# lilijiangg/AutoDiffusion

Measured on AMD Instinct MI355X. Metric: images/sec (node), ADM-G ImageNet-64 4-step DDIM, higher is better.
Workload: dtype bf16

## Files before the change

### autodiffusion_amd/csrc/adm_conv.hip

```cpp
#include <stdlib.h>

#include <type_traits>

#include "adm_common.h"
#include "adm_conv_internal.h"

namespace {

typedef __attribute__((ext_vector_type(4))) unsigned int u32x4;

constexpr int KC = 32;
constexpr int ROWB = 64 + 32;
constexpr int TI_MAX = 4;
constexpr unsigned OOB = 0x80000000u;

struct ConvK {
  const uint16_t* in0; const uint16_t* in1; const uint16_t* w; const uint16_t* res;
  const float* bias; const float* aa; const float* ab; void* out;
  float* stats;
  int stat_slabs;
  int N, H, W, C0, C1, Cout;
  int TH, TW, TI, tiles_x, tiles_y;
  int tw_shift, thw_shift;
  unsigned rcp_hpi, rcp_hw2;
  int out_mode;
  int in_up, res_up;
  int ntiles16, nblocks_n;
  int total_tiles;
  unsigned wbytes;
  int ksplit, cps;
  float* ws;
  int tap_mask, ooy, oox, slab_off;
  int nph, nbp;
  unsigned phase_bytes;
  const uint16_t* f0; const uint16_t* f1;
  int FC0, FC1;
  float out_scale;
};

template <int BM>
constexpr int stat_groups() { return BM == 128 ? 2 : 1; }

template <int NT, int HALO>
constexpr int halo_slots() { return ((HALO * 4 + NT - 1) / NT) * NT / 4; }
template <int NT, int HALO>
constexpr int conv_smem_bytes_k() { return 2 * halo_slots<NT, HALO>() * ROWB + 2 * TI_MAX * 64 * 4; }
template <int NT, int BN, int HALO, int BM>
constexpr int conv_smem_bytes() {
  constexpr int k = conv_smem_bytes_k<NT, HALO>();
  constexpr int e = BM * (BN * 2 + 16);
  constexpr int r = NT * 64;
  return (k > e ? k : e) > r ? (k > e ? k : e) : r;
}
// ... 63 lines not shown
  const int wave = __builtin_amdgcn_readfirstlane(tid >> 6);
  const int wm = wave / WN, wn = wave % WN;
  const int lc = lane & 15, lq = lane >> 4;

  const int xcd = blockIdx.x & 7;
  const int gx = (int)(gridDim.x >> 3) + (xcd < (int)(gridDim.x & 7));
  const int tcount = (p.total_tiles >> 3) + (xcd < (p.total_tiles & 7));
  const int tstart = xcd * (p.total_tiles >> 3) + min(xcd, p.total_tiles & 7);
  int tl = blockIdx.x >> 3;
  if (tl >= tcount) return;

  const int HW2 = p.TW + 2 * PAD;
  const int HPI = (p.TH + 2 * PAD) * HW2;
  const int HP = p.TI * HPI;
  const int Cin = p.C0 + p.C1;
  const int HWimg = p.H * p.W;
  const int chunks = Cin / KC;
  const int c0chunks = p.C0 / KC;
  const __amdgpu_buffer_rsrc_t rsw = __builtin_amdgcn_make_buffer_rsrc((void*)p.w, 0, p.wbytes, 0x00020000);
  const __amdgpu_buffer_rsrc_t rsb = __builtin_amdgcn_make_buffer_rsrc((void*)p.bias, 0, p.Cout * 4, 0x00020000);

  unsigned ti_pack = 0;
#pragma unroll
  for (int ps = 0; ps < PASSES; ++ps) {
    const int hp = (tid + ps * NT) >> SEGSH;
    if (hp < HP) ti_pack |= (unsigned)(hp / HPI) << (4 * ps);
  }
  const int seg = tid & (SEGP - 1);
  const int hslot = (tid >> SEGSH) * ROWB + seg * 16;

  const int alane = ((lc / p.TW) * HW2 + lc % p.TW) * ROWB + lq * 16;
  int aoff[TM];
#pragma unroll
  for (int i = 0; i < TM; ++i) {
    const int m0 = (wm * TM + i) * 16;
    const int ti = m0 / (p.TH * p.TW), rem = m0 % (p.TH * p.TW);
    aoff[i] = (ti * HPI + (rem / p.TW) * HW2) * ROWB;
  }
  const unsigned wstep = (unsigned)p.ntiles16 * 1024u;

  int nb = 0, mt = 0, img0 = 0, y0 = 0, x0 = 0;
  [[maybe_unused]] int ph = p.slab_off;
  int sp = 0, cb = 0, ce = chunks;
  __amdgpu_buffer_rsrc_t rs0 = rsw, rs1 = rsw;
  [[maybe_unused]] __amdgpu_buffer_rsrc_t rs2 = rsw, rs3 = rsw;
  int pixrel[PASSES];
  unsigned wofs[TN];
  typedef __attribute__((address_space(3))) void* lds_ptr_t;
  auto tile_origin = [&](int lt, int& nb_, int& mt_, int& img0_, int& y0_, int& x0_) {
    if (p.ksplit > 1) {
      sp = lt % p.ksplit;
      lt /= p.ksplit;
      cb = sp * p.cps;
      ce = cb + p.cps;
    }
    nb_ = lt % p.nblocks_n;
    mt_ = lt / p.nblocks_n;
    if constexpr (UPPH) {
      if (p.nph > 1) { ph = nb_ / p.nbp; nb_ -= ph * p.nbp; }
    }
    if (p.TI == 1) {
      const int per_img = p.tiles_x * p.tiles_y;
      img0_ = mt_ / per_img;
      const int r = mt_ % per_img;
      y0_ = (r / p.tiles_x) * p.TH;
      x0_ = (r % p.tiles_x) * p.TW;
    } else {
      img0_ = mt_ * p.TI;
      y0_ = 0;
      x0_ = 0;
    }
  };
  auto tile_setup = [&]() {
    const int nimg = min(p.TI, p.N - img0);
    const int Hs = p.H >> p.in_up, Ws = p.W >> p.in_up;
    rs0 = __builtin_amdgcn_make_buffer_rsrc((void*)(p.in0 + (long long)img0 * Hs * Ws * p.C0), 0, nimg * Hs * Ws * p.C0 * 2, 0x00020000);
    rs1 = __builtin_amdgcn_make_buffer_rsrc((void*)(p.C1 ? p.in1 + (long long)img0 * HWimg * p.C1 : p.in0), 0,
                                            p.C1 ? nimg * HWimg * p.C1 * 2 : 0, 0x00020000);
    if constexpr (FOLD) {
      rs2 = __builtin_amdgcn_make_buffer_rsrc((void*)(p.f0 + (long long)img0 * HWimg * p.FC0), 0, nimg * HWimg * p.FC0 * 2, 0x00020000);
      rs3 = __builtin_amdgcn_make_buffer_rsrc((void*)(p.FC1 ? p.f1 + (long long)img0 * HWimg * p.FC1 : p.f0), 0,
                                              p.FC1 ? nimg * HWimg * p.FC1 * 2 : 0, 0x00020000);
    }
    int tid_s = tid;
    asm volatile("" : "+v"(tid_s));
#pragma unroll
    for (int ps = 0; ps < PASSES; ++ps) {
      const int hp = (tid_s + ps * NT) >> SEGSH;
      const int ti = (int)(((unsigned)hp * p.rcp_hpi) >> 20), rem = hp - ti * HPI;
      const int ry = (int)(((unsigned)rem * p.rcp_hw2) >> 20), rx = rem - ry * HW2;
      const int y = y0 + ry - PAD, x = x0 + rx - PAD;
      const int ok = (int)(hp < HP) & (int)(ti < nimg) & (int)(y >= 0) & (int)(y < p.H) & (int)(x >= 0) & (int)(x < p.W);
      pixrel[ps] = ok ? (ti * Hs + (y >> p.in_up)) * Ws + (x >> p.in_up) : -1;
    }
    const int seg_s = tid_s & (SEGP - 1), lane_s = tid_s & 63;
    {
      const bool first = cb < c0chunks;
      const int cs = first ? p.C0 : p.C1, co = (first ? cb : cb - c0chunks) * KC;
      const __amdgpu_buffer_rsrc_t rsf = first ? rs0 : rs1;
#pragma unroll
      for (int ps = 0; ps < PASSES; ++ps) {
        const unsigned voff = pixrel[ps] >= 0 ? (unsigned)(pixrel[ps] * cs + co + seg_s * 8) * 2u : OOB;
        __builtin_amdgcn_raw_ptr_buffer_load_lds(rsf, (lds_ptr_t)(halo + (ps * NT + wave * 64) * 16), 16, (int)voff, 0, 0, 0);
      }
    }
    if constexpr (PRO != 0 && !ONEW) {
      if (wave < 2) {
        const int half = wave, idx = lane_s;
        const __amdgpu_buffer_rsrc_t rsa = __builtin_amdgcn_make_buffer_rsrc((void*)(half == 0 ? p.aa : p.ab), 0, p.N * Cin * 4, 0x00020000);
        const int buf = idx / (TI_MAX * (KC / 4)), ti = (idx / (KC / 4)) % TI_MAX, part = idx % (KC / 4);
        const int n = min(img0 + ti, p.N - 1);
        const unsigned voff = ti < p.TI ? (unsigned)(n * Cin + min(cb + buf, ce - 1) * KC + part * 4) * 4u : OOB;
        __builtin_amdgcn_raw_ptr_buffer_load_lds(rsa, (lds_ptr_t)(abuf + half * (2 * TI_MAX * KC)), 16, (int)voff, 0, 0, 0);
      }
    }
#pragma unroll
    for (int j = 0; j < TN; ++j) {
      const int tile = nb * (BN / 16) + wn * TN + j;
      wofs[j] = tile < p.ntiles16 ? (unsigned)((tile * 64 + lane) * 16) + (UPPH ? (unsigned)ph * p.phase_bytes : 0u) : OOB;
    }
  };

  f32x4 acc[TM][TN];

  auto halo_load = [&](int c, int ps) -> uint4 {
    const bool first = c < c0chunks;
    const int cs = first ? p.C0 : p.C1, co = (first ? c : c - c0chunks) * KC;
    const __amdgpu_buffer_rsrc_t rs = first ? rs0 : rs1;
    const unsigned voff = pixrel[ps] >= 0 ? (unsigned)(pixrel[ps] * cs + co + seg * 8) * 2u : OOB;
    return bufload16(rs, voff, 0);
  };
  [[maybe_unused]] auto halo_load_pad = [&](int c, int lastc, int ps) -> uint4 {
    const int cc = min(c, lastc);
    const bool first = cc < c0chunks;
// ... 104 lines not shown
#pragma unroll
    for (int i = 0; i < AFD; ++i) __builtin_amdgcn_sched_group_barrier(0x100, 1, 0);
#pragma unroll
    for (int i = 0; i < TM; ++i) {
      if (i + AFD < TM) __builtin_amdgcn_sched_group_barrier(0x100, 1, 0);
      __builtin_amdgcn_sched_group_barrier(0x008, TN, 0);
    }
  };

  constexpr bool NOEXIT = TM == 4 && !COLD;
  constexpr int WRING = T3 ? 3 : 4;
  uint4 wr[WRING][TN];
  constexpr int RINGN = (TAPS == 1 && NOEXIT) ? 4 : 2;
  uint4 ring[RINGN][PASSES];
  float4 bs[TN];
  auto first_loads = [&](int lq_) {
    const int last = ce - 1;
    if constexpr (T3) {
      load_w(cb * 9, wr[0]);
      load_w(cb * 9 + 1, wr[1]);
    } else {
      load_w(cb, wr[0]);
      load_w(NOEXIT ? cb + 1 : min(cb + 1, last), wr[1]);
      load_w(NOEXIT ? cb + 2 : min(cb + 2, last), wr[2]);
#pragma unroll
      for (int ps = 0; ps < PASSES; ++ps) ring[1][ps] = NOEXIT ? halo_load_pad(cb + 1, last, ps) : halo_load(min(cb + 1, last), ps);
      if constexpr (RINGN > 2) {
#pragma unroll
        for (int q = 2; q < RINGN; ++q) {
#pragma unroll
          for (int ps = 0; ps < PASSES; ++ps) ring[q][ps] = NOEXIT ? halo_load_pad(cb + q, last, ps) : halo_load(min(cb + q, last), ps);
        }
      }
    }
    if constexpr (ONEW) affine_regs(cb, img0);
#pragma unroll
    for (int j = 0; j < TN; ++j) {
      const int bch = nb * BN + (wn * TN + j) * 16 + lq_ * 4;
      const uint4 b = bufload16(rsb, (bch + 3 < p.Cout && p.ksplit <= 1) ? (unsigned)bch * 4u : OOB, 0);
      bs[j] = make_float4(__uint_as_float(b.x), __uint_as_float(b.y), __uint_as_float(b.z), __uint_as_float(b.w));
    }
  };
  auto first_park = [&]() {
    uint4 raw[PASSES];
#pragma unroll
    for (int ps = 0; ps < PASSES; ++ps) raw[ps] = *reinterpret_cast<const uint4*>(halo + (ps * NT + tid) * 16);
    __syncthreads();
#pragma unroll
    for (int ps = 0; ps < PASSES; ++ps) halo_write(raw[ps], ps, 0);
  };

  int ltile = tstart + tl;
  tile_origin(ltile, nb, mt, img0, y0, x0);
  tile_setup();
  first_loads(lq);
  __syncthreads();
  first_park();

  for (;;) {
    ADM_TSTAMP(ltile, 0);
#pragma unroll
    for (int i = 0; i < TM; ++i)
#pragma unroll
      for (int j = 0; j < TN; ++j) acc[i][j] = f32x4{bs[j].x, bs[j].y, bs[j].z, bs[j].w};
    __syncthreads();
    ADM_TSTAMP(ltile, 1);

    const int tnext = tl + gx;
    const bool more = tnext < tcount;
    if constexpr (T3 && ONEW) {
// ... 108 lines not shown
              if constexpr (RAWNEXT) raw_write(hprev, t - 1, hb ^ 1);
              else halo_write(hprev, t - 1, hb ^ 1);
            }
          }
          hprev = hcur;
          if (!UPPH || (((0x1b << ((ph >> 1) * 3 + (ph & 1))) >> t) & 1))
            mfma_tap(halo + hb * Lds::HB + ((t / 3) * HW2 + (t % 3)) * ROWB, wr[t % 3]);
        }
        __syncthreads();
      };
      for (int c = cb; c + 1 < ce; ++c) chunk(c, std::true_type{}, std::false_type{});
      if constexpr (!FOLD) {
        chunk(ce - 1, std::false_type{}, std::false_type{});
      } else {
        chunk(ce - 1, std::true_type{}, std::true_type{});
        const int fch = (p.FC0 + p.FC1) / KC, flast = fch - 1;
        const int fstep0 = chunks * 9;
        const unsigned char* const hc = halo + (HW2 + 1) * ROWB;
        constexpr int CPASS = BM * SEGP / NT;
        static_assert(CPASS * NT == BM * SEGP && CPASS <= PASSES, "centre staging: whole passes");
        int cpix[CPASS], cslot[CPASS];
        {
          int tid_c = tid;
          asm volatile("" : "+v"(tid_c));
          const int nimg_c = min(p.TI, p.N - img0);
#pragma unroll
          for (int ps = 0; ps < CPASS; ++ps) {
            const int pp = (tid_c + ps * NT) >> SEGSH;
            const int ti = pp >> p.thw_shift, rem = pp & ((1 << p.thw_shift) - 1);
            const int py = rem >> p.tw_shift, px = rem & (p.TW - 1);
            cpix[ps] = ti < nimg_c ? (ti * p.H + y0 + py) * p.W + x0 + px : -1;
            cslot[ps] = (ti * HPI + (py + 1) * HW2 + px + 1) * ROWB + (tid_c & (SEGP - 1)) * 16;
          }
        }
        auto cload = [&](int k, int ps) -> uint4 {
          const int f0chunks = p.FC0 / KC;
          const bool first = k < f0chunks;
          const int cs = first ? p.FC0 : p.FC1, co = (first ? k : k - f0chunks) * KC;
          const __amdgpu_buffer_rsrc_t rs = first ? rs2 : rs3;
          const unsigned voff = cpix[ps] >= 0 ? (unsigned)(cpix[ps] * cs + co + seg * 8) * 2u : OOB;
          return bufload16(rs, voff, 0);
        };
#pragma unroll
        for (int q = 1; q <= RINGN; ++q) {
#pragma unroll
          for (int ps = 0; ps < CPASS; ++ps) ring[q % RINGN][ps] = cload(min(q, flast), ps);
        }
        auto fbody = [&](int j, auto s_) {
          constexpr int S = decltype(s_)::value;
          if (j > flast) return;
          const int buf = (ce + j) & 1;
          load_w(fstep0 + min(j + 2, flast), wr[(S + 2) % 3]);
          mfma_tap(hc + buf * Lds::HB, wr[S % 3]);
#pragma unroll
          for (int ps = 0; ps < CPASS; ++ps) *reinterpret_cast<uint4*>(halo + (buf ^ 1) * Lds::HB + cslot[ps]) = ring[(S + 1) % RINGN][ps];
// ... 36 lines not shown
        body(c0 + 3, I1{}, I3{});
      }
    }
    ADM_TSTAMP(ltile, 2);

    const int ltile_done = ltile;
    (void)ltile_done;
    if (!COLD || (p.out_mode == 0 && p.ksplit <= 1)) {
      constexpr int EROW = BN * 2 + 16;
      constexpr int SEGS = BN / 8;
      constexpr int PR = NT / SEGS;
      constexpr int RG = BM / SGROUPS;
      constexpr int NIT = (RG + PR - 1) / PR;
      int tid_e = tid;
      asm volatile("" : "+v"(tid_e));
      const int sg = tid_e % SEGS, prow = tid_e / SEGS;
      const int gch = nb * BN + sg * 8;
      const bool act = prow < PR && gch < p.Cout;
      const int thw_mask = (1 << p.thw_shift) - 1, tw_mask = (1 << p.tw_shift) - 1;
      const long long ebase = UPPH ? (((long long)img0 * (2 * p.H) + 2 * y0 + (ph >> 1)) * (2 * p.W) + 2 * x0 + (ph & 1)) * p.Cout + gch
                                   : (((long long)img0 * p.H + y0) * p.W + x0) * p.Cout + gch;
      uint16_t* const obase = reinterpret_cast<uint16_t*>(p.out) + ebase;
      const int Hr = p.H >> p.res_up, Wr = p.W >> p.res_up;
      const uint16_t* const rbase = p.res ? p.res + (((long long)img0 * Hr + (y0 >> p.res_up)) * Wr + (x0 >> p.res_up)) * p.Cout + gch : nullptr;
      const int img0_d = img0;
      float* sdst[SGROUPS];
#pragma unroll
      for (int g = 0; g < SGROUPS; ++g) {
        const int n = img0 + ((g * RG) >> p.thw_shift);
        const int slab = p.TI == 1 ? (UPPH ? (mt % (p.tiles_x * p.tiles_y)) * 4 + ph : (mt % (p.tiles_x * p.tiles_y)) * SGROUPS + g) : 0;
        sdst[g] = (p.stats && tid_e < BN && nb * BN + tid_e < p.Cout && n < p.N)
                      ? p.stats + (((long long)n * p.stat_slabs + slab) * p.Cout + nb * BN + tid_e) * 2 : nullptr;
      }
      ADM_TSTAMP(ltile_done, 10);
#pragma unroll
      for (int j = 0; j < TN; ++j) {
        const int ch0 = (wn * TN + j) * 16 + lq * 4;
#pragma unroll
        for (int i = 0; i < TM; ++i) {
          uint2 o;
          o.x = adm_pack2(acc[i][j][0], acc[i][j][1]);
          o.y = adm_pack2(acc[i][j][2], acc[i][j][3]);
          *reinterpret_cast<uint2*>(stg + ((wm * TM + i) * 16 + lc) * EROW + ch0 * 2) = o;
        }
      }
      ADM_TSTAMP(ltile_done, 11);
      if (more) {
        tl = tnext;
        ltile = tstart + tl;
        tile_origin(ltile, nb, mt, img0, y0, x0);
        tile_setup();
      }
      int eoff[SGROUPS][NIT];
#pragma unroll
      for (int g = 0; g < SGROUPS; ++g)
#pragma unroll
        for (int k = 0; k < NIT; ++k) {
          const int ml = prow + k * PR, m = g * RG + ml;
          const int ti = m >> p.thw_shift, rem = m & thw_mask;
          eoff[g][k] = (act && ml < RG && img0_d + ti < p.N)
                           ? (UPPH ? ((rem >> p.tw_shift) * (4 * p.W) + 2 * (rem & tw_mask)) * p.Cout
                                   : ((ti * p.H + (rem >> p.tw_shift)) * p.W + (rem & tw_mask)) * p.Cout)
                           : -1;
        }
      ADM_TSTAMP(ltile_done, 12);
      uint4 rr[SGROUPS][NIT];
#pragma unroll
      for (int g = 0; g < SGROUPS; ++g)
#pragma unroll
        for (int k = 0; k < NIT; ++k) {
          rr[g][k] = make_uint4(0, 0, 0, 0);
          if (rbase && eoff[g][k] >= 0) {
            const int m = g * RG + prow + k * PR;
            const int ti = m >> p.thw_shift, rem = m & thw_mask;
            const int roff = ((ti * Hr + ((rem >> p.tw_shift) >> p.res_up)) * Wr + ((rem & tw_mask) >> p.res_up)) * p.Cout;
            rr[g][k] = *reinterpret_cast<const uint4*>(rbase + roff);
          }
        }
      [[maybe_unused]] float ga[8], gb[8];
      if constexpr (GNB) {
        const long long ao = (long long)img0_d * p.Cout + gch;
        if (act) {
          *reinterpret_cast<float4*>(ga) = *reinterpret_cast<const float4*>(p.aa + ao);
          *reinterpret_cast<float4*>(ga + 4) = *reinterpret_cast<const float4*>(p.aa + ao + 4);
          *reinterpret_cast<float4*>(gb) = *reinterpret_cast<const float4*>(p.ab + ao);
          *reinterpret_cast<float4*>(gb + 4) = *reinterpret_cast<const float4*>(p.ab + ao + 4);
        } else {
#pragma unroll
          for (int e = 0; e < 8; ++e) { ga[e] = 0.f; gb[e] = 0.f; }
        }
      }
      if (more) first_loads((tid_e & 63) >> 4);
      ADM_TSTAMP(ltile_done, 13);
      __syncthreads();
      ADM_TSTAMP(ltile_done, 3);
      if (more) first_park();
      ADM_TSTAMP(ltile_done, 4);
      typedef float f32x2 __attribute__((ext_vector_type(2)));
      f32x2 s1[SGROUPS][4], s2[SGROUPS][4];
#pragma unroll
      for (int g = 0; g < SGROUPS; ++g)
#pragma unroll
        for (int q = 0; q < 4; ++q) { s1[g][q] = f32x2{0.f, 0.f}; s2[g][q] = f32x2{0.f, 0.f}; }
#pragma unroll
      for (int g = 0; g < SGROUPS; ++g)
#pragma unroll
        for (int k = 0; k < NIT; ++k) {
          if (eoff[g][k] < 0) continue;
          uint4 v = *reinterpret_cast<const uint4*>(stg + (g * RG + prow + k * PR) * EROW + sg * 16);
          uint32_t a4[4] = {v.x, v.y, v.z, v.w};
          [[maybe_unused]] f32x2 xg[4];
          if constexpr (GNB) {
            const uint32_t r4[4] = {rr[g][k].x, rr[g][k].y, rr[g][k].z, rr[g][k].w};
#pragma unroll
            for (int q = 0; q < 4; ++q) {
              xg[q] = f32x2{adm_lo_f32(r4[q]), adm_hi_f32(r4[q])};
              const f32x2 z = f32x2{ga[2 * q], ga[2 * q + 1]} * xg[q] + f32x2{gb[2 * q], gb[2 * q + 1]};
              const f32x2 sgm = f32x2{__builtin_amdgcn_rcpf(1.0f + __builtin_amdgcn_exp2f(z.x * -1.4426950408889634f)),
                                      __builtin_amdgcn_rcpf(1.0f + __builtin_amdgcn_exp2f(z.y * -1.4426950408889634f))};
              const f32x2 t = f32x2{adm_lo_f32(a4[q]), adm_hi_f32(a4[q])} * (sgm * (1.0f + z * (1.0f - sgm)));
              a4[q] = adm_pack2(t.x, t.y);
            }
            v = make_uint4(a4[0], a4[1], a4[2], a4[3]);
          } else if (rbase) {
            const uint32_t r4[4] = {rr[g][k].x, rr[g][k].y, rr[g][k].z, rr[g][k].w};
#pragma unroll
            for (int q = 0; q < 4; ++q) {
              const f32x2 t = f32x2{adm_lo_f32(a4[q]), adm_hi_f32(a4[q])} +
                              f32x2{adm_lo_f32(r4[q]), adm_hi_f32(r4[q])};
              a4[q] = adm_pack2(t.x, t.y);
            }
            v = make_uint4(a4[0], a4[1], a4[2], a4[3]);
          }
          {
            typedef __attribute__((ext_vector_type(4))) unsigned int nt_u32x4;
            __builtin_nontemporal_store(nt_u32x4{v.x, v.y, v.z, v.w}, reinterpret_cast<nt_u32x4*>(obase + eoff[g][k]));
          }
#pragma unroll
          for (int q = 0; q < 4; ++q) {
            const f32x2 t = f32x2{adm_lo_f32(a4[q]), adm_hi_f32(a4[q])};
            s1[g][q] += t;
            if constexpr (GNB) s2[g][q] = __builtin_elementwise_fma(t, xg[q], s2[g][q]);
            else s2[g][q] = __builtin_elementwise_fma(t, t, s2[g][q]);
          }
        }
      ADM_TSTAMP(ltile_done, 5);
      if (p.stats) {
        float* red = reinterpret_cast<float*>(stg);
#pragma unroll
        for (int g = 0; g < SGROUPS; ++g) {
          __syncthreads();
          if (prow < PR) {
#pragma unroll
            for (int e = 0; e < 8; ++e) {
              red[(prow * BN + sg * 8 + e) * 2 + 0] = s1[g][e >> 1][e & 1];
              red[(prow * BN + sg * 8 + e) * 2 + 1] = s2[g][e >> 1][e & 1];
            }
          }
          __syncthreads();
          if (sdst[g]) {
            float t1 = 0.f, t2 = 0.f;
            for (int q = 0; q < PR; ++q) { t1 += red[(q * BN + tid) * 2]; t2 += red[(q * BN + tid) * 2 + 1]; }
            sdst[g][0] = t1;
            sdst[g][1] = t2;
          }
        }
      }
      ADM_TSTAMP(ltile_done, 6);
    } else if constexpr (!COLD) {
    } else if (p.ksplit > 1) {
#pragma unroll
      for (int i = 0; i < TM; ++i) {
        const int m = (wm * TM + i) * 16 + lc;
        const int ti = m >> p.thw_shift, rem = m & ((1 << p.thw_shift) - 1);
        const int n = img0 + ti, y = y0 + (rem >> p.tw_shift), x = x0 + (rem & ((1 << p.tw_shift) - 1));
        if (n >= p.N) continue;
        float* row = p.ws + ((long long)sp * p.N * HWimg + ((long long)n * p.H + y) * p.W + x) * p.Cout;
#pragma unroll
        for (int j = 0; j < TN; ++j) {
          const int ch0 = nb * BN + (wn * TN + j) * 16 + lq * 4;
          if (ch0 + 3 < p.Cout) *reinterpret_cast<float4*>(row + ch0) = make_float4(acc[i][j][0], acc[i][j][1], acc[i][j][2], acc[i][j][3]);
        }
      }
      if (more) {
        tl = tnext;
        ltile = tstart + tl;
        tile_origin(ltile, nb, mt, img0, y0, x0);
        tile_setup();
        first_loads(lq);
        __syncthreads();
        first_park();
      }
    } else {
#pragma unroll
      for (int i = 0; i < TM; ++i) {
        const int m = (wm * TM + i) * 16 + lc;
        const int ti = m >> p.thw_shift, rem = m & ((1 << p.thw_shift) - 1);
        const int n = img0 + ti, y = y0 + (rem >> p.tw_shift), x = x0 + (rem & ((1 << p.tw_shift) - 1));
        if (n >= p.N) continue;
#pragma unroll
        for (int j = 0; j < TN; ++j) {
          const int ch0 = nb * BN + (wn * TN + j) * 16 + lq * 4;
#pragma unroll
          for (int e = 0; e < 4; ++e) {
            const int ch = ch0 + e;
            if (ch >= p.Cout) continue;
            reinterpret_cast<float*>(p.out)[(((long long)n * p.Cout + ch) * p.H + y) * p.W + x] =
                (acc[i][j][e] + (ch0 + 3 < p.Cout ? 0.f : p.bias[ch])) * p.out_scale;
          }
        }
      }
      if (more) {
        tl = tnext;
        ltile = tstart + tl;
        tile_origin(ltile, nb, mt, img0, y0, x0);
        tile_setup();
              first_loads(lq);
        __syncthreads();
        first_park();
      }
    }
    if (!more) break;
  }
}

typedef __attribute__((ext_vector_type(16))) float f32x16;

template <int PRO>
__global__ void __launch_bounds__(512, 2)
conv32_kernel(const ConvK p) {
  constexpr int NT = 512, WN = 2, TM = 2, TN = 3, BN = 192, HALO = 324, WMR = 4;
  constexpr int PASSES = (HALO * 4 + NT - 1) / NT;
// ... 313 lines not shown
  __syncthreads();
  if (threadIdx.x < 128) {
    const int c = threadIdx.x >> 1, q = threadIdx.x & 1;
    float t = 0.0f;
    for (int l = 0; l < 32; ++l) t += red[l][c][q];
    if (blockIdx.x * 64 + c < cout) stats[(((long long)img * slabs + slab) * cout + blockIdx.x * 64 + c) * 2 + q] = t;
  }
}

template <int WM, int WN, int TM, int TN, int OCC, int TAPS, int HALO, int PRO, int KS, bool COLD>
int launch_conv_p(const ConvK& k, int m_tiles, hipStream_t s) {
  constexpr int NT = 64 * WM * WN;
  constexpr int BN = WN * TN * 16;
  constexpr int smem = ConvLds<NT, BN, HALO, WM * TM * 16>::BYTES;
  static_assert(smem <= 160 * 1024, "conv_kernel LDS map exceeds the CU's 160 KB");
  static int percu_dev[64] = {}, ncu_dev[64] = {};
  int dev = 0;
  (void)hipGetDevice(&dev);
  int& per_cu_d = percu_dev[dev & 63];
  int& ncu_d = ncu_dev[dev & 63];
  const void* fn = reinterpret_cast<const void*>(&conv_kernel<WM, WN, TM, TN, OCC, TAPS, HALO, PRO, KS, COLD>);
  if (per_cu_d == 0) {
    hipError_t e = hipFuncSetAttribute(fn, hipFuncAttributeMaxDynamicSharedMemorySize, smem);
    if (e != hipSuccess) ADM_FAIL((int)e, "adm_conv: hipFuncSetAttribute: %s", hipGetErrorString(e));
    int per_cu = 0, ncu = 0;
    e = hipOccupancyMaxActiveBlocksPerMultiprocessor(&per_cu, fn, NT, smem);
    if (e != hipSuccess || per_cu <= 0) ADM_FAIL((int)e, "adm_conv: block of %d threads / %d B LDS is not launchable", NT, smem);
    e = hipDeviceGetAttribute(&ncu, hipDeviceAttributeMultiprocessorCount, dev);
    if (e != hipSuccess || ncu <= 0) ADM_FAIL((int)e, "adm_conv: hipDeviceGetAttribute: %s", hipGetErrorString(e));
    ncu_d = ncu;
    per_cu_d = per_cu;
  }
  const int slots = per_cu_d * adm_stream_cus((void*)s, ncu_d);
  ConvK kk = k;
  kk.nbp = (k.Cout + BN - 1) / BN;
  kk.nblocks_n = kk.nbp * (k.nph > 1 ? k.nph : 1);
  const long long tiles = (long long)m_tiles * kk.nblocks_n * (k.ksplit > 1 ? k.ksplit : 1);
  ADM_REQUIRE(tiles < (1ll << 31), ADM_E_SHAPE, "adm_conv: too many tiles");
  kk.total_tiles = (int)tiles;
  unsigned blocks = (unsigned)(tiles < slots ? tiles : slots);
#ifdef ADM_CONV_TIMING
  if (const char* e = getenv("ADM_CONV_MAX_BLOCKS")) { const unsigned cap = (unsigned)atoi(e); if (cap > 0 && cap < blocks) blocks = cap; }
#endif
  hipLaunchKernelGGL((conv_kernel<WM, WN, TM, TN, OCC, TAPS, HALO, PRO, KS, COLD>), dim3(blocks), dim3(NT), smem, s, kk);
  return adm_check_launch("adm_conv");
}

template <int WM, int WN, int TM, int TN, int OCC, int TAPS, int HALO, int KS, bool COLD>
int launch_conv(const ConvK& k, int prologue, int m_tiles, hipStream_t s) {
  switch (prologue) {
    case 0: return launch_conv_p<WM, WN, TM, TN, OCC, TAPS, HALO, 0, KS, COLD>(k, m_tiles, s);
    case 1: return launch_conv_p<WM, WN, TM, TN, OCC, TAPS, HALO, 1, KS, COLD>(k, m_tiles, s);
    case 3:
// ... 283 lines not shown
```

Before: 794.2.

## Cut conv tile-switch scalar overhead with magic division, kernarg reloads and buffer stores

Replaces integer divisions in the tile decode with host-computed magic multipliers, and turns hot-path divisions into shifts. Kernel arguments are re-read from the kernarg segment at tile switches instead of being held live across the main loop. Epilogue output, residual and stats writes go through buffer resources with 32-bit offsets instead of 64-bit pointer arithmetic. The aim is to lower register pressure and the instruction count between tiles, at the cost of new host-side range checks and 2 GiB per-tile window limits.

```diff
diff --git a/autodiffusion_amd/csrc/adm_conv.hip b/autodiffusion_amd/csrc/adm_conv.hip
--- a/autodiffusion_amd/csrc/adm_conv.hip
+++ b/autodiffusion_amd/csrc/adm_conv.hip
@@ -36,7 +36,12 @@
   const uint16_t* f0; const uint16_t* f1;
   int FC0, FC1;
   float out_scale;
+  unsigned m_ksplit, m_nblocks, m_nbp, m_perimg, m_tilesx;
 };
+
+typedef const __attribute__((address_space(4))) ConvK* conv_kargs_t;
+
+__device__ __forceinline__ int mdiv(int x, unsigned m) { return (int)(((unsigned long long)(unsigned)x * m) >> 31); }
 
 template <int BM>
 constexpr int stat_groups() { return BM == 128 ? 2 : 1; }
@@ -130,28 +135,31 @@
   const int HPI = (p.TH + 2 * PAD) * HW2;
   const int HP = p.TI * HPI;
   const int Cin = p.C0 + p.C1;
-  const int HWimg = p.H * p.W;
   const int chunks = Cin / KC;
   const int c0chunks = p.C0 / KC;
   const __amdgpu_buffer_rsrc_t rsw = __builtin_amdgcn_make_buffer_rsrc((void*)p.w, 0, p.wbytes, 0x00020000);
-  const __amdgpu_buffer_rsrc_t rsb = __builtin_amdgcn_make_buffer_rsrc((void*)p.bias, 0, p.Cout * 4, 0x00020000);
+  auto kargs = []() -> conv_kargs_t {
+    conv_kargs_t q = (conv_kargs_t)__builtin_amdgcn_kernarg_segment_ptr();
+    asm volatile("" : "+s"(q));
+    return q;
+  };
 
   unsigned ti_pack = 0;
 #pragma unroll
   for (int ps = 0; ps < PASSES; ++ps) {
     const int hp = (tid + ps * NT) >> SEGSH;
-    if (hp < HP) ti_pack |= (unsigned)(hp / HPI) << (4 * ps);
+    if (hp < HP) ti_pack |= (((unsigned)hp * p.rcp_hpi) >> 20) << (4 * ps);
   }
   const int seg = tid & (SEGP - 1);
   const int hslot = (tid >> SEGSH) * ROWB + seg * 16;
 
-  const int alane = ((lc / p.TW) * HW2 + lc % p.TW) * ROWB + lq * 16;
+  const int alane = ((lc >> p.tw_shift) * HW2 + (lc & (p.TW - 1))) * ROWB + lq * 16;
   int aoff[TM];
 #pragma unroll
   for (int i = 0; i < TM; ++i) {
     const int m0 = (wm * TM + i) * 16;
-    const int ti = m0 / (p.TH * p.TW), rem = m0 % (p.TH * p.TW);
-    aoff[i] = (ti * HPI + (rem / p.TW) * HW2) * ROWB;
+    const int ti = m0 >> p.thw_shift, rem = m0 & ((1 << p.thw_shift) - 1);
+    aoff[i] = (ti * HPI + (rem >> p.tw_shift) * HW2) * ROWB;
   }
   const unsigned wstep = (unsigned)p.ntiles16 * 1024u;
 
@@ -163,56 +171,64 @@
   int pixrel[PASSES];
   unsigned wofs[TN];
   typedef __attribute__((address_space(3))) void* lds_ptr_t;
-  auto tile_origin = [&](int lt, int& nb_, int& mt_, int& img0_, int& y0_, int& x0_) {
-    if (p.ksplit > 1) {
-      sp = lt % p.ksplit;
-      lt /= p.ksplit;
-      cb = sp * p.cps;
-      ce = cb + p.cps;
-    }
-    nb_ = lt % p.nblocks_n;
-    mt_ = lt / p.nblocks_n;
+  auto tile_origin = [&](const conv_kargs_t q, int lt, int& nb_, int& mt_, int& img0_, int& y0_, int& x0_) {
+    if constexpr (COLD) {
+      if (q->ksplit > 1) {
+        const int l2 = mdiv(lt, q->m_ksplit);
+        sp = lt - l2 * q->ksplit;
+        lt = l2;
+        cb = sp * q->cps;
+        ce = cb + q->cps;
+      }
+    }
+    mt_ = mdiv(lt, q->m_nblocks);
+    nb_ = lt - mt_ * q->nblocks_n;
     if constexpr (UPPH) {
-      if (p.nph > 1) { ph = nb_ / p.nbp; nb_ -= ph * p.nbp; }
-    }
-    if (p.TI == 1) {
-      const int per_img = p.tiles_x * p.tiles_y;
-      img0_ = mt_ / per_img;
-      const int r = mt_ % per_img;
-      y0_ = (r / p.tiles_x) * p.TH;
-      x0_ = (r % p.tiles_x) * p.TW;
+      if (q->nph > 1) { ph = mdiv(nb_, q->m_nbp); nb_ -= ph * q->nbp; }
+    }
+    if (q->TI == 1) {
+      const int tx = q->tiles_x;
+      img0_ = mdiv(mt_, q->m_perimg);
+      const int r = mt_ - img0_ * (tx * q->tiles_y);
+      const int ty = mdiv(r, q->m_tilesx);
+      y0_ = ty * q->TH;
+      x0_ = (r - ty * tx) * q->TW;
     } else {
-      img0_ = mt_ * p.TI;
+      img0_ = mt_ * q->TI;
       y0_ = 0;
       x0_ = 0;
     }
   };
-  auto tile_setup = [&]() {
-    const int nimg = min(p.TI, p.N - img0);
-    const int Hs = p.H >> p.in_up, Ws = p.W >> p.in_up;
-    rs0 = __builtin_amdgcn_make_buffer_rsrc((void*)(p.in0 + (long long)img0 * Hs * Ws * p.C0), 0, nimg * Hs * Ws * p.C0 * 2, 0x00020000);
-    rs1 = __builtin_amdgcn_make_buffer_rsrc((void*)(p.C1 ? p.in1 + (long long)img0 * HWimg * p.C1 : p.in0), 0,
-                                            p.C1 ? nimg * HWimg * p.C1 * 2 : 0, 0x00020000);
+  auto tile_setup = [&](const conv_kargs_t q) {
+    const int TI = q->TI, N = q->N, H = q->H, W = q->W, C0 = q->C0, C1 = q->C1, in_up = q->in_up;
+    const int HW2 = q->TW + 2 * PAD, HPI = (q->TH + 2 * PAD) * HW2, HP = TI * HPI, Cin = C0 + C1, HWimg = H * W;
+    const int nimg = min(TI, N - img0);
+    const int Hs = H >> in_up, Ws = W >> in_up;
+    rs0 = __builtin_amdgcn_make_buffer_rsrc((void*)(q->in0 + (long long)img0 * Hs * Ws * C0), 0, nimg * Hs * Ws * C0 * 2, 0x00020000);
+    rs1 = __builtin_amdgcn_make_buffer_rsrc((void*)(C1 ? q->in1 + (long long)img0 * HWimg * C1 : q->in0), 0,
+                                            C1 ? nimg * HWimg * C1 * 2 : 0, 0x00020000);
     if constexpr (FOLD) {
-      rs2 = __builtin_amdgcn_make_buffer_rsrc((void*)(p.f0 + (long long)img0 * HWimg * p.FC0), 0, nimg * HWimg * p.FC0 * 2, 0x00020000);
-      rs3 = __builtin_amdgcn_make_buffer_rsrc((void*)(p.FC1 ? p.f1 + (long long)img0 * HWimg * p.FC1 : p.f0), 0,
-                                              p.FC1 ? nimg * HWimg * p.FC1 * 2 : 0, 0x00020000);
+      const int FC0 = q->FC0, FC1 = q->FC1;
+      rs2 = __builtin_amdgcn_make_buffer_rsrc((void*)(q->f0 + (long long)img0 * HWimg * FC0), 0, nimg * HWimg * FC0 * 2, 0x00020000);
+      rs3 = __builtin_amdgcn_make_buffer_rsrc((void*)(FC1 ? q->f1 + (long long)img0 * HWimg * FC1 : q->f0), 0,
+                                              FC1 ? nimg * HWimg * FC1 * 2 : 0, 0x00020000);
     }
     int tid_s = tid;
     asm volatile("" : "+v"(tid_s));
+    const unsigned rcp_hpi = q->rcp_hpi, rcp_hw2 = q->rcp_hw2;
 #pragma unroll
     for (int ps = 0; ps < PASSES; ++ps) {
       const int hp = (tid_s + ps * NT) >> SEGSH;
-      const int ti = (int)(((unsigned)hp * p.rcp_hpi) >> 20), rem = hp - ti * HPI;
-      const int ry = (int)(((unsigned)rem * p.rcp_hw2) >> 20), rx = rem - ry * HW2;
+      const int ti = (int)(((unsigned)hp * rcp_hpi) >> 20), rem = hp - ti * HPI;
+      const int ry = (int)(((unsigned)rem * rcp_hw2) >> 20), rx = rem - ry * HW2;
       const int y = y0 + ry - PAD, x = x0 + rx - PAD;
-      const int ok = (int)(hp < HP) & (int)(ti < nimg) & (int)(y >= 0) & (int)(y < p.H) & (int)(x >= 0) & (int)(x < p.W);
-      pixrel[ps] = ok ? (ti * Hs + (y >> p.in_up)) * Ws + (x >> p.in_up) : -1;
+      const int ok = (int)(hp < HP) & (int)(ti < nimg) & (int)(y >= 0) & (int)(y < H) & (int)(x >= 0) & (int)(x < W);
+      pixrel[ps] = ok ? (ti * Hs + (y >> in_up)) * Ws + (x >> in_up) : -1;
     }
     const int seg_s = tid_s & (SEGP - 1), lane_s = tid_s & 63;
     {
       const bool first = cb < c0chunks;
-      const int cs = first ? p.C0 : p.C1, co = (first ? cb : cb - c0chunks) * KC;
+      const int cs = first ? C0 : C1, co = (first ? cb : cb - c0chunks) * KC;
       const __amdgpu_buffer_rsrc_t rsf = first ? rs0 : rs1;
 #pragma unroll
       for (int ps = 0; ps < PASSES; ++ps) {
@@ -223,17 +239,17 @@
     if constexpr (PRO != 0 && !ONEW) {
       if (wave < 2) {
         const int half = wave, idx = lane_s;
-        const __amdgpu_buffer_rsrc_t rsa = __builtin_amdgcn_make_buffer_rsrc((void*)(half == 0 ? p.aa : p.ab), 0, p.N * Cin * 4, 0x00020000);
+        const __amdgpu_buffer_rsrc_t rsa = __builtin_amdgcn_make_buffer_rsrc((void*)(half == 0 ? q->aa : q->ab), 0, N * Cin * 4, 0x00020000);
         const int buf = idx / (TI_MAX * (KC / 4)), ti = (idx / (KC / 4)) % TI_MAX, part = idx % (KC / 4);
-        const int n = min(img0 + ti, p.N - 1);
-        const unsigned voff = ti < p.TI ? (unsigned)(n * Cin + min(cb + buf, ce - 1) * KC + part * 4) * 4u : OOB;
+        const int n = min(img0 + ti, N - 1);
+        const unsigned voff = ti < TI ? (unsigned)(n * Cin + min(cb + buf, ce - 1) * KC + part * 4) * 4u : OOB;
         __builtin_amdgcn_raw_ptr_buffer_load_lds(rsa, (lds_ptr_t)(abuf + half * (2 * TI_MAX * KC)), 16, (int)voff, 0, 0, 0);
       }
     }
 #pragma unroll
     for (int j = 0; j < TN; ++j) {
       const int tile = nb * (BN / 16) + wn * TN + j;
-      wofs[j] = tile < p.ntiles16 ? (unsigned)((tile * 64 + lane) * 16) + (UPPH ? (unsigned)ph * p.phase_bytes : 0u) : OOB;
+      wofs[j] = tile < q->ntiles16 ? (unsigned)((tile * 64 + lane) * 16) + (UPPH ? (unsigned)ph * q->phase_bytes : 0u) : OOB;
     }
   };
 
@@ -368,7 +384,7 @@
   constexpr int RINGN = (TAPS == 1 && NOEXIT) ? 4 : 2;
   uint4 ring[RINGN][PASSES];
   float4 bs[TN];
-  auto first_loads = [&](int lq_) {
+  auto first_loads = [&](const conv_kargs_t q, int lq_) {
     const int last = ce - 1;
     if constexpr (T3) {
       load_w(cb * 9, wr[0]);
@@ -388,10 +404,13 @@
       }
     }
     if constexpr (ONEW) affine_regs(cb, img0);
+    const int Cout = q->Cout;
+    const bool nosplit = !COLD || q->ksplit <= 1;
+    const __amdgpu_buffer_rsrc_t rsb = __builtin_amdgcn_make_buffer_rsrc((void*)q->bias, 0, Cout * 4, 0x00020000);
 #pragma unroll
     for (int j = 0; j < TN; ++j) {
       const int bch = nb * BN + (wn * TN + j) * 16 + lq_ * 4;
-      const uint4 b = bufload16(rsb, (bch + 3 < p.Cout && p.ksplit <= 1) ? (unsigned)bch * 4u : OOB, 0);
+      const uint4 b = bufload16(rsb, (bch + 3 < Cout && nosplit) ? (unsigned)bch * 4u : OOB, 0);
       bs[j] = make_float4(__uint_as_float(b.x), __uint_as_float(b.y), __uint_as_float(b.z), __uint_as_float(b.w));
     }
   };
@@ -405,9 +424,12 @@
   };
 
   int ltile = tstart + tl;
-  tile_origin(ltile, nb, mt, img0, y0, x0);
-  tile_setup();
-  first_loads(lq);
+  {
+    const conv_kargs_t q = kargs();
+    tile_origin(q, ltile, nb, mt, img0, y0, x0);
+    tile_setup(q);
+    first_loads(q, lq);
+  }
   __syncthreads();
   first_park();
 
@@ -546,31 +568,35 @@
         chunk(ce - 1, std::false_type{}, std::false_type{});
       } else {
         chunk(ce - 1, std::true_type{}, std::true_type{});
-        const int fch = (p.FC0 + p.FC1) / KC, flast = fch - 1;
+        const conv_kargs_t qf = kargs();
+        const int FC0 = qf->FC0, FC1 = qf->FC1;
+        const int fch = (FC0 + FC1) / KC, flast = fch - 1;
         const int fstep0 = chunks * 9;
         const unsigned char* const hc = halo + (HW2 + 1) * ROWB;
         constexpr int CPASS = BM * SEGP / NT;
         static_assert(CPASS * NT == BM * SEGP && CPASS <= PASSES, "centre staging: whole passes");
         int cpix[CPASS], cslot[CPASS];
+        int tid_c = tid;
+        asm volatile("" : "+v"(tid_c));
+        const int seg_c = tid_c & (SEGP - 1);
         {
-          int tid_c = tid;
-          asm volatile("" : "+v"(tid_c));
-          const int nimg_c = min(p.TI, p.N - img0);
+          const int nimg_c = min(qf->TI, qf->N - img0);
+          const int thw_shift = qf->thw_shift, tw_shift = qf->tw_shift, H = qf->H, W = qf->W;
 #pragma unroll
           for (int ps = 0; ps < CPASS; ++ps) {
             const int pp = (tid_c + ps * NT) >> SEGSH;
-            const int ti = pp >> p.thw_shift, rem = pp & ((1 << p.thw_shift) - 1);
-            const int py = rem >> p.tw_shift, px = rem & (p.TW - 1);
-            cpix[ps] = ti < nimg_c ? (ti * p.H + y0 + py) * p.W + x0 + px : -1;
-            cslot[ps] = (ti * HPI + (py + 1) * HW2 + px + 1) * ROWB + (tid_c & (SEGP - 1)) * 16;
+            const int ti = pp >> thw_shift, rem = pp & ((1 << thw_shift) - 1);
+            const int py = rem >> tw_shift, px = rem & ((1 << tw_shift) - 1);
+            cpix[ps] = ti < nimg_c ? (ti * H + y0 + py) * W + x0 + px : -1;
+            cslot[ps] = (ti * HPI + (py + 1) * HW2 + px + 1) * ROWB + seg_c * 16;
           }
         }
         auto cload = [&](int k, int ps) -> uint4 {
-          const int f0chunks = p.FC0 / KC;
+          const int f0chunks = FC0 / KC;
           const bool first = k < f0chunks;
-          const int cs = first ? p.FC0 : p.FC1, co = (first ? k : k - f0chunks) * KC;
+          const int cs = first ? FC0 : FC1, co = (first ? k : k - f0chunks) * KC;
           const __amdgpu_buffer_rsrc_t rs = first ? rs2 : rs3;
-          const unsigned voff = cpix[ps] >= 0 ? (unsigned)(cpix[ps] * cs + co + seg * 8) * 2u : OOB;
+          const unsigned voff = cpix[ps] >= 0 ? (unsigned)(cpix[ps] * cs + co + seg_c * 8) * 2u : OOB;
           return bufload16(rs, voff, 0);
         };
 #pragma unroll
@@ -637,23 +663,38 @@
       constexpr int NIT = (RG + PR - 1) / PR;
       int tid_e = tid;
       asm volatile("" : "+v"(tid_e));
+      const conv_kargs_t q = kargs();
+      const int Cout = q->Cout, W = q->W, tw_shift = q->tw_shift, thw_shift = q->thw_shift, res_up = q->res_up;
+      const uint16_t* const resp = q->res;
       const int sg = tid_e % SEGS, prow = tid_e / SEGS;
       const int gch = nb * BN + sg * 8;
-      const bool act = prow < PR && gch < p.Cout;
-      const int thw_mask = (1 << p.thw_shift) - 1, tw_mask = (1 << p.tw_shift) - 1;
-      const long long ebase = UPPH ? (((long long)img0 * (2 * p.H) + 2 * y0 + (ph >> 1)) * (2 * p.W) + 2 * x0 + (ph & 1)) * p.Cout + gch
-                                   : (((long long)img0 * p.H + y0) * p.W + x0) * p.Cout + gch;
-      uint16_t* const obase = reinterpret_cast<uint16_t*>(p.out) + ebase;
-      const int Hr = p.H >> p.res_up, Wr = p.W >> p.res_up;
-      const uint16_t* const rbase = p.res ? p.res + (((long long)img0 * Hr + (y0 >> p.res_up)) * Wr + (x0 >> p.res_up)) * p.Cout + gch : nullptr;
+      const bool act = prow < PR && gch < Cout;
+      const int tw_mask = (1 << tw_shift) - 1;
+      const int nimg_d = min(q->TI, q->N - img0);
+      const int Wr = W >> res_up;
+      __amdgpu_buffer_rsrc_t rso, rsr;
+      {
+        const int H = q->H;
+        const int img_e = (UPPH ? 4 : 1) * H * W * Cout;
+        const int org = UPPH ? ((2 * y0 + (ph >> 1)) * (2 * W) + 2 * x0 + (ph & 1)) * Cout : (y0 * W + x0) * Cout;
+        rso = __builtin_amdgcn_make_buffer_rsrc(reinterpret_cast<uint16_t*>(q->out) + ((long long)img0 * img_e + org), 0,
+                                                (int)((unsigned)(nimg_d * img_e - org) * 2u), 0x00020000);
+        const int rimg_e = (H >> res_up) * Wr * Cout, rorg = ((y0 >> res_up) * Wr + (x0 >> res_up)) * Cout;
+        rsr = __builtin_amdgcn_make_buffer_rsrc(resp ? (void*)(resp + ((long long)img0 * rimg_e + rorg)) : q->out, 0,
+                                                resp ? (int)((unsigned)(nimg_d * rimg_e - rorg) * 2u) : 0, 0x00020000);
+      }
       const int img0_d = img0;
-      float* sdst[SGROUPS];
-#pragma unroll
-      for (int g = 0; g < SGROUPS; ++g) {
-        const int n = img0 + ((g * RG) >> p.thw_shift);
-        const int slab = p.TI == 1 ? (UPPH ? (mt % (p.tiles_x * p.tiles_y)) * 4 + ph : (mt % (p.tiles_x * p.tiles_y)) * SGROUPS + g) : 0;
-        sdst[g] = (p.stats && tid_e < BN && nb * BN + tid_e < p.Cout && n < p.N)
-                      ? p.stats + (((long long)n * p.stat_slabs + slab) * p.Cout + nb * BN + tid_e) * 2 : nullptr;
+      unsigned soff[SGROUPS];
+      {
+        const int slabs = q->stat_slabs;
+        const bool one = q->TI == 1;
+        const int rt = one ? mt - img0 * (q->tiles_x * q->tiles_y) : 0;
+#pragma unroll
+        for (int g = 0; g < SGROUPS; ++g) {
+          const int ng = (g * RG) >> thw_shift;
+          const int slab = one ? (UPPH ? rt * 4 + ph : rt * SGROUPS + g) : 0;
+          soff[g] = (tid_e < BN && nb * BN + tid_e < Cout && ng < nimg_d) ? (unsigned)((ng * slabs + slab) * Cout + nb * BN + tid_e) * 8u : OOB;
+        }
       }
       ADM_TSTAMP(ltile_done, 10);
 #pragma unroll
@@ -671,49 +712,54 @@
       if (more) {
         tl = tnext;
         ltile = tstart + tl;
-        tile_origin(ltile, nb, mt, img0, y0, x0);
-        tile_setup();
-      }
-      int eoff[SGROUPS][NIT];
+        tile_origin(q, ltile, nb, mt, img0, y0, x0);
+        tile_setup(q);
+      }
+      unsigned eoff[SGROUPS][NIT], roff[SGROUPS][NIT];
 #pragma unroll
       for (int g = 0; g < SGROUPS; ++g)
 #pragma unroll
         for (int k = 0; k < NIT; ++k) {
           const int ml = prow + k * PR, m = g * RG + ml;
-          const int ti = m >> p.thw_shift, rem = m & thw_mask;
-          eoff[g][k] = (act && ml < RG && img0_d + ti < p.N)
-                           ? (UPPH ? ((rem >> p.tw_shift) * (4 * p.W) + 2 * (rem & tw_mask)) * p.Cout
-                                   : ((ti * p.H + (rem >> p.tw_shift)) * p.W + (rem & tw_mask)) * p.Cout)
-                           : -1;
-        }
+          const int my = m >> tw_shift, mx = m & tw_mask;
+          const bool ok = act && ml < RG && (m >> thw_shift) < nimg_d;
+          const int pix = UPPH ? my * (4 * W) + 2 * mx : my * W + mx;
+          eoff[g][k] = ok ? (unsigned)(pix * Cout + gch) * 2u : OOB;
+          roff[g][k] = eoff[g][k];
+        }
+      if (res_up) {
+#pragma unroll
+        for (int g = 0; g < SGROUPS; ++g)
+#pragma unroll
+          for (int k = 0; k < NIT; ++k) {
+            const int m = g * RG + prow + k * PR;
+            const int pix = ((m >> tw_shift) >> 1) * Wr + ((m & tw_mask) >> 1);
+            roff[g][k] = eoff[g][k] != OOB ? (unsigned)(pix * Cout + gch) * 2u : OOB;
+          }
+      }
       ADM_TSTAMP(ltile_done, 12);
       uint4 rr[SGROUPS][NIT];
 #pragma unroll
       for (int g = 0; g < SGROUPS; ++g)
 #pragma unroll
-        for (int k = 0; k < NIT; ++k) {
-          rr[g][k] = make_uint4(0, 0, 0, 0);
-          if (rbase && eoff[g][k] >= 0) {
-            const int m = g * RG + prow + k * PR;
-            const int ti = m >> p.thw_shift, rem = m & thw_mask;
-            const int roff = ((ti * Hr + ((rem >> p.tw_shift) >> p.res_up)) * Wr + ((rem & tw_mask) >> p.res_up)) * p.Cout;
-            rr[g][k] = *reinterpret_cast<const uint4*>(rbase + roff);
-          }
-        }
+        for (int k = 0; k < NIT; ++k) rr[g][k] = make_uint4(0, 0, 0, 0);
+      if (resp) {
+#pragma unroll
+        for (int g = 0; g < SGROUPS; ++g)
+#pragma unroll
+          for (int k = 0; k < NIT; ++k) rr[g][k] = bufload16(rsr, roff[g][k], 0);
+      }
       [[maybe_unused]] float ga[8], gb[8];
       if constexpr (GNB) {
-        const long long ao = (long long)img0_d * p.Cout + gch;
-        if (act) {
-          *reinterpret_cast<float4*>(ga) = *reinterpret_cast<const float4*>(p.aa + ao);
-          *reinterpret_cast<float4*>(ga + 4) = *reinterpret_cast<const float4*>(p.aa + ao + 4);
-          *reinterpret_cast<float4*>(gb) = *reinterpret_cast<const float4*>(p.ab + ao);
-          *reinterpret_cast<float4*>(gb + 4) = *reinterpret_cast<const float4*>(p.ab + ao + 4);
-        } else {
-#pragma unroll
-          for (int e = 0; e < 8; ++e) { ga[e] = 0.f; gb[e] = 0.f; }
-        }
-      }
-      if (more) first_loads((tid_e & 63) >> 4);
+        const __amdgpu_buffer_rsrc_t rga = __builtin_amdgcn_make_buffer_rsrc((void*)(q->aa + (long long)img0_d * Cout), 0, Cout * 4, 0x00020000);
+        const __amdgpu_buffer_rsrc_t rgb = __builtin_amdgcn_make_buffer_rsrc((void*)(q->ab + (long long)img0_d * Cout), 0, Cout * 4, 0x00020000);
+        const unsigned go = act ? (unsigned)gch * 4u : OOB;
+        const uint4 a0 = bufload16(rga, go, 0), a1 = bufload16(rga, go + 16u, 0), b0 = bufload16(rgb, go, 0), b1 = bufload16(rgb, go + 16u, 0);
+        const uint32_t au[8] = {a0.x, a0.y, a0.z, a0.w, a1.x, a1.y, a1.z, a1.w}, bu[8] = {b0.x, b0.y, b0.z, b0.w, b1.x, b1.y, b1.z, b1.w};
+#pragma unroll
+        for (int e = 0; e < 8; ++e) { ga[e] = __uint_as_float(au[e]); gb[e] = __uint_as_float(bu[e]); }
+      }
+      if (more) first_loads(q, (tid_e & 63) >> 4);
       ADM_TSTAMP(ltile_done, 13);
       __syncthreads();
       ADM_TSTAMP(ltile_done, 3);
@@ -729,7 +775,7 @@
       for (int g = 0; g < SGROUPS; ++g)
 #pragma unroll
         for (int k = 0; k < NIT; ++k) {
-          if (eoff[g][k] < 0) continue;
+          if ((k + 1) * PR > RG && eoff[g][k] == OOB) continue;
           uint4 v = *reinterpret_cast<const uint4*>(stg + (g * RG + prow + k * PR) * EROW + sg * 16);
           uint32_t a4[4] = {v.x, v.y, v.z, v.w};
           [[maybe_unused]] f32x2 xg[4];
@@ -745,7 +791,7 @@
               a4[q] = adm_pack2(t.x, t.y);
             }
             v = make_uint4(a4[0], a4[1], a4[2], a4[3]);
-          } else if (rbase) {
+          } else if (resp) {
             const uint32_t r4[4] = {rr[g][k].x, rr[g][k].y, rr[g][k].z, rr[g][k].w};
 #pragma unroll
             for (int q = 0; q < 4; ++q) {
@@ -755,10 +801,7 @@
             }
             v = make_uint4(a4[0], a4[1], a4[2], a4[3]);
           }
-          {
-            typedef __attribute__((ext_vector_type(4))) unsigned int nt_u32x4;
-            __builtin_nontemporal_store(nt_u32x4{v.x, v.y, v.z, v.w}, reinterpret_cast<nt_u32x4*>(obase + eoff[g][k]));
-          }
+          __builtin_amdgcn_raw_buffer_store_b128(u32x4{v.x, v.y, v.z, v.w}, rso, (int)eoff[g][k], 0, 2);
 #pragma unroll
           for (int q = 0; q < 4; ++q) {
             const f32x2 t = f32x2{adm_lo_f32(a4[q]), adm_hi_f32(a4[q])};
@@ -768,8 +811,12 @@
           }
         }
       ADM_TSTAMP(ltile_done, 5);
-      if (p.stats) {
+      const conv_kargs_t qs = kargs();
+      if (float* const statp = qs->stats) {
         float* red = reinterpret_cast<float*>(stg);
+        const int sbytes = qs->stat_slabs * qs->Cout * 8;
+        const __amdgpu_buffer_rsrc_t rss = __builtin_amdgcn_make_buffer_rsrc(reinterpret_cast<char*>(statp) + (long long)img0_d * sbytes, 0,
+                                                                             nimg_d * sbytes, 0x00020000);
 #pragma unroll
         for (int g = 0; g < SGROUPS; ++g) {
           __syncthreads();
@@ -781,11 +828,11 @@
             }
           }
           __syncthreads();
-          if (sdst[g]) {
+          if (soff[g] != OOB) {
             float t1 = 0.f, t2 = 0.f;
-            for (int q = 0; q < PR; ++q) { t1 += red[(q * BN + tid) * 2]; t2 += red[(q * BN + tid) * 2 + 1]; }
-            sdst[g][0] = t1;
-            sdst[g][1] = t2;
+            for (int r = 0; r < PR; ++r) { t1 += red[(r * BN + tid) * 2]; t2 += red[(r * BN + tid) * 2 + 1]; }
+            typedef __attribute__((ext_vector_type(2))) unsigned int u32x2;
+            __builtin_amdgcn_raw_buffer_store_b64(u32x2{__float_as_uint(t1), __float_as_uint(t2)}, rss, (int)soff[g], 0, 0);
           }
         }
       }
@@ -798,7 +845,7 @@
         const int ti = m >> p.thw_shift, rem = m & ((1 << p.thw_shift) - 1);
         const int n = img0 + ti, y = y0 + (rem >> p.tw_shift), x = x0 + (rem & ((1 << p.tw_shift) - 1));
         if (n >= p.N) continue;
-        float* row = p.ws + ((long long)sp * p.N * HWimg + ((long long)n * p.H + y) * p.W + x) * p.Cout;
+        float* row = p.ws + ((long long)sp * p.N * (p.H * p.W) + ((long long)n * p.H + y) * p.W + x) * p.Cout;
 #pragma unroll
         for (int j = 0; j < TN; ++j) {
           const int ch0 = nb * BN + (wn * TN + j) * 16 + lq * 4;
@@ -808,9 +855,10 @@
       if (more) {
         tl = tnext;
         ltile = tstart + tl;
-        tile_origin(ltile, nb, mt, img0, y0, x0);
-        tile_setup();
-        first_loads(lq);
+        const conv_kargs_t q = kargs();
+        tile_origin(q, ltile, nb, mt, img0, y0, x0);
+        tile_setup(q);
+        first_loads(q, lq);
         __syncthreads();
         first_park();
       }
@@ -836,9 +884,10 @@
       if (more) {
         tl = tnext;
         ltile = tstart + tl;
-        tile_origin(ltile, nb, mt, img0, y0, x0);
-        tile_setup();
-              first_loads(lq);
+        const conv_kargs_t q = kargs();
+        tile_origin(q, ltile, nb, mt, img0, y0, x0);
+        tile_setup(q);
+        first_loads(q, lq);
         __syncthreads();
         first_park();
       }
@@ -1182,6 +1231,22 @@
   constexpr int BN = WN * TN * 16;
   constexpr int smem = ConvLds<NT, BN, HALO, WM * TM * 16>::BYTES;
   static_assert(smem <= 160 * 1024, "conv_kernel LDS map exceeds the CU's 160 KB");
+  ConvK kk = k;
+  kk.nbp = (k.Cout + BN - 1) / BN;
+  kk.nblocks_n = kk.nbp * (k.nph > 1 ? k.nph : 1);
+  const int ksp = k.ksplit > 1 ? k.ksplit : 1, per_img = k.tiles_x * k.tiles_y;
+  const long long tiles = (long long)m_tiles * kk.nblocks_n * ksp;
+  ADM_REQUIRE(COLD || ksp == 1, ADM_E_ARG, "adm_conv: split-K runs on the COLD instantiations");
+  const int dmax = ksp > kk.nblocks_n ? (ksp > per_img ? ksp : per_img) : (kk.nblocks_n > per_img ? kk.nblocks_n : per_img);
+  ADM_REQUIRE(tiles * dmax < (1ll << 31), ADM_E_SHAPE, "adm_conv: %lld tiles (x %d) exceed the tile decode's 32-bit range", tiles, dmax);
+  auto magic = [](int d) { return (unsigned)(((1ull << 31) + (unsigned)d - 1) / (unsigned)d); };
+  kk.m_ksplit = magic(ksp); kk.m_nblocks = magic(kk.nblocks_n); kk.m_nbp = magic(kk.nbp);
+  kk.m_perimg = magic(per_img); kk.m_tilesx = magic(k.tiles_x);
+  if (k.out_mode == 0 && ksp == 1) {
+    const long long img_bytes = (long long)k.TI * k.H * k.W * k.Cout * 2 * (TAPS == 4 ? 4 : 1);
+    ADM_REQUIRE(img_bytes < (1ll << 31) && (long long)k.TI * k.stat_slabs * k.Cout * 8 < (1ll << 31), ADM_E_SHAPE,
+                "adm_conv: %d x %d x %d output images exceed the epilogue's 2 GiB window per tile", k.H, k.W, k.Cout);
+  }
   static int percu_dev[64] = {}, ncu_dev[64] = {};
   int dev = 0;
   (void)hipGetDevice(&dev);
@@ -1200,11 +1265,6 @@
     per_cu_d = per_cu;
   }
   const int slots = per_cu_d * adm_stream_cus((void*)s, ncu_d);
-  ConvK kk = k;
-  kk.nbp = (k.Cout + BN - 1) / BN;
-  kk.nblocks_n = kk.nbp * (k.nph > 1 ? k.nph : 1);
-  const long long tiles = (long long)m_tiles * kk.nblocks_n * (k.ksplit > 1 ? k.ksplit : 1);
-  ADM_REQUIRE(tiles < (1ll << 31), ADM_E_SHAPE, "adm_conv: too many tiles");
   kk.total_tiles = (int)tiles;
   unsigned blocks = (unsigned)(tiles < slots ? tiles : slots);
 #ifdef ADM_CONV_TIMING
diff --git a/profiles/conv_tile_switch/count_tile.py b/profiles/conv_tile_switch/count_tile.py
--- /dev/null
+++ b/profiles/conv_tile_switch/count_tile.py
@@ -0,0 +1,67 @@
+#!/usr/bin/env python3
+import re
+import subprocess
+import sys
+
+
+def kernels(path):
+    name, body = None, []
+    for line in open(path):
+        m = re.match(r"^(_Z\w+):", line)
+        if m:
+            name, body = m.group(1), []
+            continue
+        if name is None:
+            continue
+        body.append(line)
+        if line.lstrip().startswith(".end_amdhsa_kernel"):
+            yield name, body
+            name = None
+
+
+def count(body):
+    ins = [l.split("//")[0].split(";")[0].strip() for l in body]
+    ins = [l for l in ins if l and not l.startswith(".") and not l.endswith(":")]
+    end = next((i for i, l in enumerate(ins) if l.startswith("s_endpgm")), len(ins) - 1)
+    ins = ins[:end + 1]
+    mf = [i for i, l in enumerate(ins) if l.startswith("v_mfma")]
+    if not mf:
+        return None
+    before, region, after = ins[:mf[0]], ins[mf[0]:mf[-1] + 1], ins[mf[-1] + 1:]
+
+    def n(where, *prefixes):
+        return sum(1 for l in where if l.startswith(prefixes))
+    vgpr = next((int(m.group(1)) for l in body for m in [re.search(r"\.amdhsa_next_free_vgpr\s+(\d+)", l)] if m), -1)
+    return dict(before=len(before), inside=len(region), after=len(after), mfma=len(mf),
+                addr64=n(after, "v_mad_u64_u32", "v_lshl_add_u64"), mul_lo=n(after, "v_mul_lo_u32"),
+                execbr=n(after, "s_and_saveexec", "s_cbranch_exec"), readlane=n(after, "v_readlane_b32"),
+                mul_hi=n(after, "s_mul_hi_u32"), rcp=n(ins, "v_rcp_iflag_f32"), nop=n(ins, "s_nop"),
+                writelane_before=n(before, "v_writelane_b32"),
+                in_readlane=n(region, "v_readlane_b32"), in_addr64=n(region, "v_mad_u64_u32", "v_lshl_add_u64"),
+                in_execbr=n(region, "s_and_saveexec", "s_cbranch_exec"),
+                bufst=n(after, "buffer_store"), globst=n(after, "global_store"),
+                vgpr=vgpr, scratch=n(ins, "scratch_"))
+
+
+def main():
+    path, want = sys.argv[1], sys.argv[2:]
+    rows = []
+    for name, body in kernels(path):
+        dem = subprocess.run(["c++filt", name], capture_output=True, text=True).stdout.strip()
+        dem = re.sub(r"^void ", "", dem).replace("(anonymous namespace)::", "").split("(")[0]
+        if want and not any(w in dem for w in want):
+            continue
+        c = count(body)
+        if c:
+            rows.append((dem, c))
+    print("symbol | instructions before / inside / after the MFMA region (MFMAs) | after: 64-bit address math, v_mul_lo_u32, "
+          "exec-mask pairs, v_readlane, s_mul_hi_u32, buffer / global stores | whole symbol: v_rcp_iflag, s_nop | v_writelane before | "
+          "inside: v_readlane, 64-bit address math, exec-mask pairs | vgprs | scratch instructions")
+    for dem, c in sorted(rows):
+        print(f"{dem} | {c['before']} / {c['inside']} / {c['after']} ({c['mfma']}) | {c['addr64']} {c['mul_lo']} {c['execbr']} "
+              f"{c['readlane']} {c['mul_hi']} {c['bufst']}/{c['globst']} | {c['rcp']} {c['nop']} | {c['writelane_before']} | "
+              f"{c['in_readlane']} {c['in_addr64']} {c['in_execbr']} | {c['vgpr']} | {c['scratch']}")
+
+
+if __name__ == "__main__":
+    main()
```

New measurement: 801.1, median of 6. About the same (+0.9%).
